# liuyuan-pal/Gen6D

Hardware: AMD Instinct MI355X
Metric: query images/sec (detect+select+3x refine), 64 ref views (higher is better)
Workload: dtype f32

## Files before the change

gen6d_amd/csrc/corr_fft.hip:

```cpp
#include "g6d_common.h"
#include "corr_fft_plan.h"

namespace {

constexpr int T = 32, HB = T / 2 + 1;
constexpr int CG = 32;
constexpr int RS = HB * 2 * CG;
constexpr int FWD_LDS = T * RS * 4;
constexpr int NT = 512;

struct CfftSeg { const float* in; float* out; int ld_in, ld_out; };
struct CfftParams {
  cfft::Plan plan;
  CfftSeg seg[cfft::MAX_SEG];
  int Cin;
  float* X;
  const float* Y;
};

__host__ __device__ constexpr double tw_c8(int k) {
  constexpr double c[9] = {1.0, 0.98078528040323043, 0.92387953251128674, 0.83146961230254524, 0.70710678118654752,
                           0.55557023301960218, 0.38268343236508977, 0.19509032201612825, 0.0};
  return c[k];
}
__host__ __device__ constexpr double tw_cos(int k) { return k <= 8 ? tw_c8(k) : -tw_c8(16 - k); }
__host__ __device__ constexpr double tw_sin(int k) { return k <= 8 ? tw_c8(8 - k) : tw_c8(k - 8); }
__host__ __device__ constexpr int br5(int k) { return ((k & 1) << 4) | ((k & 2) << 2) | (k & 4) | ((k & 8) >> 2) | ((k & 16) >> 4); }

__device__ __forceinline__ void fft32(float (&re)[T], float (&im)[T]) {
#pragma unroll
  for (int h = 16; h >= 1; h >>= 1) {
#pragma unroll
    for (int b = 0; b < T; b += 2 * h) {
#pragma unroll
      for (int j = 0; j < h; ++j) {
        const int k = j * (16 / h);
        const float c = (float)tw_cos(k), s = (float)tw_sin(k);
        const float ur = re[b + j], ui = im[b + j], vr = re[b + j + h], vi = im[b + j + h];
        re[b + j] = ur + vr; im[b + j] = ui + vi;
        const float dr = ur - vr, di = ui - vi;
        if (k == 0) { re[b + j + h] = dr; im[b + j + h] = di; }
        else if (k == 8) { re[b + j + h] = di; im[b + j + h] = -dr; }
        else { re[b + j + h] = dr * c + di * s; im[b + j + h] = di * c - dr * s; }
      }
    }
  }
}

__global__ __launch_bounds__(NT) void corrfft_fwd_kernel(const CfftParams p) {
  extern __shared__ __attribute__((aligned(16))) float L[];
  const int tid = threadIdx.x, c = tid & (CG - 1), g = tid >> 5;
  const int tile = blockIdx.x, c0 = blockIdx.y * CG;
  const cfft::Tile t = cfft::tile_of(p.plan, tile);
  const cfft::SegPlan& sp = p.plan.seg[t.seg];
  const CfftSeg& sg = p.seg[t.seg];
  const int H = sp.H, W = sp.W, wy = cfft::window_y(p.plan, t), wx = cfft::window_x(p.plan, t);
  float re[T], im[T];
  {
    const int ya = wy + 2 * g, yb = ya + 1;
    const bool oka = ya >= 0 && ya < H, okb = yb >= 0 && yb < H;
    const float* img = sg.in + (size_t)t.n * H * W * sg.ld_in + c0 + c;
#pragma unroll
    for (int x = 0; x < T; ++x) {
      const int xx = wx + x;
      const bool okx = xx >= 0 && xx < W;
      re[x] = oka && okx ? img[((size_t)ya * W + xx) * sg.ld_in] : 0.f;
      im[x] = okb && okx ? img[((size_t)yb * W + xx) * sg.ld_in] : 0.f;
    }
  }
  fft32(re, im);
  {
    float* ra = L + (2 * g) * RS + c;
    float* rb = ra + RS;
#pragma unroll
    for (int k = 0; k < HB; ++k) {
      const int a = br5(k), b = br5((T - k) & (T - 1));
      ra[k * 64] = 0.5f * (re[a] + re[b]); ra[k * 64 + 32] = 0.5f * (im[a] - im[b]);
      rb[k * 64] = 0.5f * (im[a] + im[b]); rb[k * 64 + 32] = 0.5f * (re[b] - re[a]);
    }
  }
  __syncthreads();
  if (g == 0) {
#pragma unroll
    for (int y = 0; y < T; ++y) { re[y] = L[y * RS + c]; im[y] = L[y * RS + 16 * 64 + c]; }
  } else {
#pragma unroll
    for (int y = 0; y < T; ++y) { re[y] = L[y * RS + g * 64 + c]; im[y] = L[y * RS + g * 64 + 32 + c]; }
  }
  fft32(re, im);
  if (g == 0) {
#pragma unroll
    for (int k = 0; k < T; ++k) {
      const int a = br5(k), b = br5((T - k) & (T - 1));
      L[k * RS + c] = 0.5f * (re[a] + re[b]); L[k * RS + 32 + c] = 0.5f * (im[a] - im[b]);
      L[k * RS + 16 * 64 + c] = 0.5f * (im[a] + im[b]); L[k * RS + 16 * 64 + 32 + c] = 0.5f * (re[b] - re[a]);
    }
  } else {
#pragma unroll
    for (int k = 0; k < T; ++k) { L[k * RS + g * 64 + c] = re[br5(k)]; L[k * RS + g * 64 + 32 + c] = im[br5(k)]; }
  }
  __syncthreads();
  const size_t tiles = (size_t)p.plan.tiles;
#pragma unroll 1
  for (int i = tid; i < T * HB * 16; i += NT) {
    const int q = i & 7, pl = (i >> 3) & 1, bin = i >> 4, ky = bin / HB, kx = bin - ky * HB;
    const f32x4 v = *reinterpret_cast<const f32x4*>(L + ky * RS + kx * 64 + pl * 32 + 4 * q);
    *reinterpret_cast<f32x4*>(p.X + (((size_t)bin * tiles + tile) * 2 + pl) * p.Cin + c0 + 4 * q) = v;
  }
}

constexpr int GEMM_NT = 128, GEMM_BM = 128;
struct CfftGemm { const float* X; const float* B; float* Y; int M, bins, K2, mblocks; };

__global__ __launch_bounds__(GEMM_NT) void corrfft_gemm_kernel(const CfftGemm p) {
  const int b = blockIdx.x, xcd = b & 7, s = b >> 3;
  const int bin = xcd + 8 * (s / p.mblocks), mb = s % p.mblocks;
  if (bin >= p.bins) return;
  const int lane = threadIdx.x & 63, wv = threadIdx.x >> 6, r = lane & 31, h = lane >> 5;
  const int m0 = mb * GEMM_BM + wv * 64;
  if (m0 >= p.M) return;
  const int K2 = p.K2;
  const float* A0 = p.X + ((size_t)bin * p.M + min(m0 + r, p.M - 1)) * K2 + 16 * h;
  const float* A1 = p.X + ((size_t)bin * p.M + min(m0 + 32 + r, p.M - 1)) * K2 + 16 * h;
  const float* Bp = p.B + ((size_t)bin * K2 + 16 * h) * 64 + r;
  f32x16 acc[2][2];
#pragma unroll
  for (int i = 0; i < 2; ++i)
#pragma unroll
    for (int n = 0; n < 2; ++n)
#pragma unroll
      for (int q = 0; q < 16; ++q) acc[i][n][q] = 0.f;
  f32x4 a0[2][4], a1[2][4];
  float b0[2][16], b1[2][16];
  auto load = [&](int k0, f32x4 (&x0)[4], f32x4 (&x1)[4], float (&y0)[16], float (&y1)[16]) {
#pragma unroll
    for (int j = 0; j < 4; ++j) {
      x0[j] = *reinterpret_cast<const f32x4*>(A0 + k0 + 4 * j);
      x1[j] = *reinterpret_cast<const f32x4*>(A1 + k0 + 4 * j);
    }
#pragma unroll
    for (int e = 0; e < 16; ++e) { y0[e] = Bp[(size_t)(k0 + e) * 64]; y1[e] = Bp[(size_t)(k0 + e) * 64 + 32]; }
  };
  auto mac = [&](const f32x4 (&x0)[4], const f32x4 (&x1)[4], const float (&y0)[16], const float (&y1)[16]) {
#pragma unroll
    for (int e = 0; e < 16; ++e) {
      const float u0 = x0[e >> 2][e & 3], u1 = x1[e >> 2][e & 3];
      acc[0][0] = __builtin_amdgcn_mfma_f32_32x32x2f32(u0, y0[e], acc[0][0], 0, 0, 0);
      acc[0][1] = __builtin_amdgcn_mfma_f32_32x32x2f32(u0, y1[e], acc[0][1], 0, 0, 0);
      acc[1][0] = __builtin_amdgcn_mfma_f32_32x32x2f32(u1, y0[e], acc[1][0], 0, 0, 0);
      acc[1][1] = __builtin_amdgcn_mfma_f32_32x32x2f32(u1, y1[e], acc[1][1], 0, 0, 0);
    }
  };
  load(0, a0[0], a1[0], b0[0], b1[0]);
#pragma unroll 1
  for (int k0 = 0; k0 < K2; k0 += 64) {
    load(k0 + 32, a0[1], a1[1], b0[1], b1[1]);
    mac(a0[0], a1[0], b0[0], b1[0]);
    if (k0 + 64 < K2) load(k0 + 64, a0[0], a1[0], b0[0], b1[0]);
    mac(a0[1], a1[1], b0[1], b1[1]);
  }
  float* Yb = p.Y + (size_t)bin * p.M * 64 + r;
#pragma unroll
  for (int i = 0; i < 2; ++i)
#pragma unroll
    for (int q = 0; q < 16; ++q) {
      const int row = m0 + 32 * i + (q & 3) + 8 * (q >> 2) + 4 * h;
      if (row < p.M) { Yb[(size_t)row * 64] = acc[i][0][q]; Yb[(size_t)row * 64 + 32] = acc[i][1][q]; }
    }
}

constexpr int INV_ROWS = 18;
constexpr int INV_LDS = INV_ROWS * RS * 4;

__global__ __launch_bounds__(NT) void corrfft_inv_kernel(const CfftParams p) {
  extern __shared__ __attribute__((aligned(16))) float L[];
  const int tid = threadIdx.x, r = tid & (CG - 1), g = tid >> 5;
  const int tile = blockIdx.x, V = p.plan.V;
  const cfft::Tile t = cfft::tile_of(p.plan, tile);
  const cfft::SegPlan& sp = p.plan.seg[t.seg];
  const CfftSeg& sg = p.seg[t.seg];
  const size_t bs = (size_t)p.plan.tiles * 64;
  const float* Y = p.Y + (size_t)tile * 64 + r;
  float re[T], im[T];
  if (g == 0) {
#pragma unroll
    for (int k = 0; k < T; ++k) {
      const float* y0 = Y + (size_t)(k * HB) * bs;
      const float* y16 = Y + (size_t)(k * HB + 16) * bs;
      re[k] = y0[0] - y16[32]; im[k] = y0[32] + y16[0];
    }
  } else {
#pragma unroll
    for (int k = 0; k < T; ++k) {
      const float* y = Y + (size_t)(k * HB + g) * bs;
      re[k] = y[0]; im[k] = y[32];
    }
  }
  fft32(im, re);
  if (g == 0) {
#pragma unroll
    for (int y = 0; y < INV_ROWS; ++y) {
      L[y * RS + r] = re[br5(y)]; L[y * RS + 32 + r] = 0.f;
      L[y * RS + 16 * 64 + r] = im[br5(y)]; L[y * RS + 16 * 64 + 32 + r] = 0.f;
    }
  } else {
#pragma unroll
    for (int y = 0; y < INV_ROWS; ++y) { L[y * RS + g * 64 + r] = re[br5(y)]; L[y * RS + g * 64 + 32 + r] = im[br5(y)]; }
  }
  __syncthreads();
  if (2 * g >= V) return;
  const float* ga = L + (2 * g) * RS + r;
  const float* gb = ga + RS;
#pragma unroll
  for (int k = 0; k < HB; ++k) {
    const float ar = ga[k * 64], ai = ga[k * 64 + 32], br = gb[k * 64], bi = gb[k * 64 + 32];
    re[k] = ar - bi; im[k] = ai + br;
    if (k > 0 && k < T / 2) { re[T - k] = ar + bi; im[T - k] = br - ai; }
  }
  fft32(im, re);
  const int H = sp.H, W = sp.W, ya = t.y0 + 2 * g;
  const float sc = 1.f / (T * T);
  float* o = sg.out + (size_t)t.n * H * W * sg.ld_out + r;
#pragma unroll
  for (int x = 0; x < INV_ROWS; ++x) {
    const int xx = t.x0 + x;
    if (x < V && xx < W) {
      if (ya < H) o[((size_t)ya * W + xx) * sg.ld_out] = re[br5(x)] * sc;
      if (ya + 1 < H) o[((size_t)(ya + 1) * W + xx) * sg.ld_out] = im[br5(x)] * sc;
    }
  }
}

int cfft_params(CfftParams& p, const char* what, const G6dCorrSeg* segs, int nseg, int C, int k, int Tw, bool fwd) {
  if (!segs || nseg < 1 || nseg > cfft::MAX_SEG) { g6d_set_error("corr_fft: 1..4 segments expected"); return G6D_EINVAL; }
  if (Tw != T || k != 15) { g6d_set_error("corr_fft: the kernels are built for T = 32, k = 15"); return G6D_EINVAL; }
  int N[cfft::MAX_SEG], H[cfft::MAX_SEG], W[cfft::MAX_SEG];
  for (int i = 0; i < nseg; ++i) { N[i] = segs[i].N; H[i] = segs[i].H; W[i] = segs[i].W; }
  if (!cfft::make_plan(p.plan, Tw, k, nseg, N, H, W) || p.plan.V > INV_ROWS || (p.plan.V & 1)) { g6d_set_error("corr_fft: bad map sizes"); return G6D_EINVAL; }
  for (int i = 0; i < nseg; ++i) {
    const G6dCorrSeg& s = segs[i];
    const bool ok = fwd ? (s.in && s.ld_in >= C && !(s.ld_in & 3) && g6d_aligned16(s.in)) : (s.out && s.ld_out >= C);
    if (!ok) { g6d_set_error(what); return G6D_EINVAL; }
    p.seg[i] = CfftSeg{s.in, s.out, s.ld_in, s.ld_out};
  }
  return G6D_OK;
}
}

extern "C" int g6d_corr_fft_plan(const G6dCorrSeg* segs, int nseg, int Cin, int Cout, int k, int Tw, int64_t* out) {
  if (!segs || !out || nseg < 1 || nseg > cfft::MAX_SEG || Cin < 1 || Cout < 1) { g6d_set_error("corr_fft_plan: bad arguments"); return G6D_EINVAL; }
  int N[cfft::MAX_SEG], H[cfft::MAX_SEG], W[cfft::MAX_SEG], one[cfft::MAX_SEG];
  for (int i = 0; i < nseg; ++i) { N[i] = segs[i].N; H[i] = segs[i].H; W[i] = segs[i].W; one[i] = 1; }
  cfft::Plan p, q;
  if (!cfft::make_plan(p, Tw, k, nseg, N, H, W) || !cfft::make_plan(q, Tw, k, nseg, one, H, W)) { g6d_set_error("corr_fft_plan: bad sizes"); return G6D_EINVAL; }
  out[0] = p.tiles; out[1] = p.bins; out[2] = p.V;
  out[3] = cfft::spectrum_bytes(Tw, p.tiles, Cin); out[4] = cfft::product_bytes(Tw, p.tiles, Cout); out[5] = cfft::filter_bytes(Tw, Cin, Cout);
  out[6] = q.tiles;
  out[7] = cfft::chunk_queries(Tw, q.tiles, Cin, 1 << 16);
  return G6D_OK;
}

extern "C" int g6d_corr_fft_fwd(const G6dCorrSeg* segs, int nseg, int Cin, int k, int Tw, float* X, g6d_stream_t stream) {
  CfftParams p = {};
  if (int rc = cfft_params(p, "corr_fft_fwd: bad segment (fp32 channels-last maps, 16-byte aligned, ld_in % 4 == 0)", segs, nseg, Cin, k, Tw, true)) return rc;
  if (!X || !g6d_aligned16(X) || Cin % CG) { g6d_set_error("corr_fft_fwd: Cin % 32 == 0 and an aligned spectrum expected"); return G6D_EINVAL; }
  if (cfft::spectrum_bytes(Tw, p.plan.tiles, Cin) >= (1ll << 31)) { g6d_set_error("corr_fft_fwd: spectrum beyond 2 GB, launch fewer queries"); return G6D_ENOSPC; }
  p.Cin = Cin; p.X = X;
  g6d_allow_lds(reinterpret_cast<const void*>(&corrfft_fwd_kernel), FWD_LDS);
  hipLaunchKernelGGL(corrfft_fwd_kernel, dim3(p.plan.tiles, Cin / CG), dim3(NT), FWD_LDS, static_cast<hipStream_t>(stream), p);
  return g6d_check_launch("corr_fft_fwd");
}

extern "C" int g6d_corr_fft_gemm(const float* X, const float* B, float* Y, int tiles, int Cin, int Cout, int Tw, g6d_stream_t stream) {
  if (!X || !B || !Y || tiles < 1 || Tw != T || Cout != 32 || Cin < 32 || Cin % 32 || !g6d_aligned16(X)) {
    g6d_set_error("corr_fft_gemm: T = 32, 32 references, Cin % 32 == 0 expected"); return G6D_EINVAL;
  }
  if (cfft::spectrum_bytes(Tw, tiles, Cin) >= (1ll << 31)) { g6d_set_error("corr_fft_gemm: spectrum beyond 2 GB"); return G6D_ENOSPC; }
  CfftGemm p = {X, B, Y, tiles, cfft::bins(Tw), 2 * Cin, (tiles + GEMM_BM - 1) / GEMM_BM};
  static_assert(cfft::bins(T) % 8 == 0, "blocks of a bin stay on one XCD");
  hipLaunchKernelGGL(corrfft_gemm_kernel, dim3(p.bins * p.mblocks), dim3(GEMM_NT), 0, static_cast<hipStream_t>(stream), p);
  return g6d_check_launch("corr_fft_gemm");
}

extern "C" int g6d_corr_fft_inv(const G6dCorrSeg* segs, int nseg, int Cout, int k, int Tw, const float* Y, g6d_stream_t stream) {
  CfftParams p = {};
  if (int rc = cfft_params(p, "corr_fft_inv: bad segment (ld_out >= 32)", segs, nseg, Cout, k, Tw, false)) return rc;
  if (!Y || Cout != CG) { g6d_set_error("corr_fft_inv: 32 references expected"); return G6D_EINVAL; }
  p.Y = Y;
  g6d_allow_lds(reinterpret_cast<const void*>(&corrfft_inv_kernel), INV_LDS);
  hipLaunchKernelGGL(corrfft_inv_kernel, dim3(p.plan.tiles), dim3(NT), INV_LDS, static_cast<hipStream_t>(stream), p);
  return g6d_check_launch("corr_fft_inv");
}
```

gen6d_amd/csrc/corr_fft_plan.h:

```cpp
#pragma once
#include <stdint.h>

#if defined(__HIPCC__) || defined(__CUDACC__)
#define CFFT_HD __host__ __device__ inline
#else
#define CFFT_HD inline
#endif

namespace cfft {

constexpr int MAX_SEG = 4;

CFFT_HD constexpr bool valid_tk(int T, int K) { return (T == 32 || T == 64) && K >= 1 && (K & 1) && K < T; }
CFFT_HD constexpr int valid_side(int T, int K) { return T - K + 1; }
CFFT_HD constexpr int bins(int T) { return T * (T / 2 + 1); }

struct SegPlan { int H, W, N, tiles_x, tiles_y, tpi, tile0; };
struct Plan {
  int T, K, V, bins, nseg, tiles;
  SegPlan seg[MAX_SEG];
};
struct Tile { int seg, n, y0, x0; };

CFFT_HD int ceil_div(int a, int b) { return (a + b - 1) / b; }

CFFT_HD bool make_plan(Plan& p, int T, int K, int nseg, const int* N, const int* H, const int* W) {
  if (!valid_tk(T, K) || nseg < 1 || nseg > MAX_SEG) return false;
  p.T = T; p.K = K; p.V = valid_side(T, K); p.bins = bins(T); p.nseg = nseg;
  int64_t tiles = 0;
  for (int i = 0; i < nseg; ++i) {
    if (N[i] < 1 || H[i] < 1 || W[i] < 1) return false;
    SegPlan& s = p.seg[i];
    s.H = H[i]; s.W = W[i]; s.N = N[i];
    s.tiles_x = ceil_div(W[i], p.V); s.tiles_y = ceil_div(H[i], p.V);
    s.tpi = s.tiles_x * s.tiles_y; s.tile0 = (int)tiles;
    tiles += (int64_t)s.tpi * N[i];
    if (tiles >= (1ll << 24)) return false;
  }
  p.tiles = (int)tiles;
  return true;
}

CFFT_HD Tile tile_of(const Plan& p, int t) {
  int si = 0;
  for (int i = 1; i < p.nseg; ++i) if (t >= p.seg[i].tile0) si = i;
  const SegPlan& s = p.seg[si];
  const int l = t - s.tile0, n = l / s.tpi, r = l - n * s.tpi, ty = r / s.tiles_x, tx = r - ty * s.tiles_x;
  return {si, n, ty * p.V, tx * p.V};
}
CFFT_HD int window_y(const Plan& p, const Tile& t) { return t.y0 - p.K / 2; }
CFFT_HD int window_x(const Plan& p, const Tile& t) { return t.x0 - p.K / 2; }

CFFT_HD int64_t spectrum_bytes(int T, int64_t tiles, int Cin) { return (int64_t)bins(T) * tiles * 2 * Cin * 4; }
CFFT_HD int64_t product_bytes(int T, int64_t tiles, int R) { return (int64_t)bins(T) * tiles * 2 * R * 4; }
CFFT_HD int64_t filter_bytes(int T, int Cin, int R) { return (int64_t)bins(T) * 2 * Cin * 2 * R * 4; }

CFFT_HD int chunk_queries(int T, int tiles_per_query, int Cin, int want) {
  int q = want;
  while (q > 0 && spectrum_bytes(T, (int64_t)q * tiles_per_query, Cin) >= (1ll << 31)) --q;
  return q;
}

}
```

gen6d_amd/ops.py:

```python
import ctypes as C
import math

import numpy as np
import torch

from . import lib as _lib

_WS = {}
WORKSPACE_BYTES = 96 << 20
MATH_MODE = 0
_MATH_NAMES = {"fp32": 0, "f32": 0, "bf16": 1, "fp16": 2, "f16": 2, 0: 0, 1: 1, 2: 2, None: 0}


class math_mode:

    def __init__(self, mode, inherit_if_none=False):
        self.mode = None if (mode is None and inherit_if_none) else _MATH_NAMES[mode]

    def __enter__(self):
        global MATH_MODE
        self.prev = MATH_MODE
        if self.mode is not None:
            MATH_MODE = self.mode
        return self
# ... 808 lines not shown
def l2norm_split16(x, mode, rng=None):
    _need_gpu(x)
    if x.dtype != torch.float32 or not x.is_contiguous() or x.dim() != 4:
        raise ValueError("l2norm_split16: a dense float32 [N,H,W,C] tap expected")
    N, H, W, Cc = x.shape
    out, ra = _pair_out("l2norm_split16", (N, H, W), Cc, mode, x.device, rng)
    _timed_hbm("l2norm_split16", 4.0 * x.numel() + 2.0 * out.numel(), lambda: _lib.check(_lib.load().g6d_l2norm_split16(
        _ptr(x), Cc, N * H * W, Cc, _ptr(out), int(mode), ra, _stream()), "g6d_l2norm_split16"))
    return _wrap(out, rng)


def vgg_conv1_pool_nhwc16(x, w_oihw, bias, out=None, norm=None, mode=None, rng=None):
    _need_gpu(x, w_oihw, bias)
    mode = MATH_MODE if mode is None else mode
    if mode not in _T16:
        raise RuntimeError("vgg_conv1_pool_nhwc16: mode 1 (bf16), 2 (fp16) or 3 (fp16 pairs)")
    N, Cin, H, W = x.shape
    Cout = w_oihw.shape[0]
    out, ra = _pair_out("vgg_conv1_pool_nhwc16", (N, H // 2, W // 2), Cout, mode, x.device, rng, out)
    mean = std = None
    if norm is not None:
        mean, std = (C.c_float * 3)(*norm[0]), (C.c_float * 3)(*norm[1])
    _lib.check(_lib.load().g6d_vgg_conv1_pool_nhwc16_ex(_ptr(x.contiguous()), N, H, W, _ptr(w_oihw.contiguous()), _ptr(bias), Cin, Cout,
                                                        mean, std, _ptr(out), int(mode), ra, _stream()),
               "g6d_vgg_conv1_pool_nhwc16")
    return _wrap(out, rng)


def conv16_direct_multi(xs, filt, bias, relu=True, full=None, pool=None, kd=1, stats=None, rows_per_group=0, out_full=None, rng=None):
    xs, table_in, slot_in = _pair_inputs(xs)
    if (table_in is not None or rng is not None) and filt.mode != 3:
        raise ValueError("conv16_direct_multi: ranges apply to pairs (mode 3) only")
    ra = _range_arg(table_in, slot_in, rng)
    _need_gpu(filt.data, *xs)
    mode = filt.mode
    t16 = _T16[mode]
    Cout, taps, Cin = filt.Cout, filt.taps, filt.Cin
    if taps != 9 * kd:
        raise ValueError("conv16_direct_multi: filters / kd mismatch")
    pair = mode == 3
    code = {None: 0, "t16": 3 if pair else 1, torch.float32: 2}
    if full not in code or pool not in code:
        raise ValueError('conv16_direct_multi: output types are None, torch.float32 or "t16"')
    segs = (_lib.G6dConv16Seg * len(xs))()
    fulls, pools, flops, sizes, nbytes = [], [], 0.0, [], 2.0 * filt.data.numel()
    nd = (4 if kd == 1 else 5) + (1 if pair else 0)
    for i, x in enumerate(xs):
        if x.dtype != t16 or not x.is_contiguous() or x.dim() != nd or x.shape[-1] != Cin or (pair and x.shape[-2] != 2):
            raise ValueError(f"conv16_direct_multi: input {i} must be a dense {t16} channels-last tensor with {Cin} channels{' in hi / lo planes' if pair else ''}")
        N, D, H, W = (x.shape[0], 1, x.shape[1], x.shape[2]) if kd == 1 else tuple(x.shape[:4])
        lead = (N, H, W) if kd == 1 else (N, D, H, W)

        def alloc(kind, lead_):
            if kind is None:
                return None
            if kind == "t16":
                return torch.empty(lead_ + ((2, Cout) if pair else (Cout,)), dtype=t16, device=x.device)
            return torch.empty(lead_ + (Cout,), dtype=torch.float32, device=x.device)
        q = alloc(pool, (N, H // 2, W // 2))
        ld_f = None
        if out_full is not None:
            f = out_full[i]
            want_t = torch.float32 if full is torch.float32 else t16
            nel = N * D * H * W * Cout * (2 if (pair and full == "t16") else 1)
            if full is None or f.dtype != want_t or f.numel() != nel or f.stride(-1) != 1:
                raise ValueError("conv16_direct_multi: out_full must hold the outputs' type and size")
            if not f.is_contiguous():
                ld_f = f.stride(-2)
                if full is not torch.float32 or f.shape[-1] != Cout or any(f.stride(d) != f.stride(d + 1) * f.shape[d + 1] for d in range(f.dim() - 2)):
                    raise ValueError("conv16_direct_multi: a strided out_full must be an fp32 channel slice of dense rows")
        else:
            f = alloc(full, lead)
        fulls.append(f); pools.append(q)
        ld = lambda t_: (2 * Cout if t_.dtype != torch.float32 and pair else Cout)
        segs[i] = _lib.G6dConv16Seg(in_=x.data_ptr(), out_full=f.data_ptr() if f is not None else None,
                                    out_pool=q.data_ptr() if q is not None else None, N=N, D=D, H=H, W=W, ld_in=(2 if pair else 1) * Cin,
                                    ld_full=(ld_f or ld(f)) if f is not None else 0, ld_pool=ld(q) if q is not None else 0)
        flops += 2.0 * N * D * H * W * Cout * taps * Cin
        nbytes += x.numel() * 2.0 + sum(t.numel() * t.element_size() for t in (f, q) if t is not None)
        sizes.append("x".join(str(v) for v in lead))
    _timed(PROFILE is not None,
           lambda: _lib.check(_lib.load().g6d_conv16_direct_multi_ex(
               segs, len(xs), Cin, _ptr(filt.data), int(filt.layout), float(filt.acc_scale), _ptr(bias), Cout, int(kd), int(bool(relu)), code[full],
               code[pool], int(mode), _ptr(stats), int(rows_per_group), ra, _stream()), "g6d_conv16_direct_multi"),
           lambda e0, e1: PROFILE.append((flops, e0, e1, f"{'conv16x3' if pair else 'conv16'} direct in={'+'.join(sizes)}x{Cin} out={Cout} k={'3x' if kd == 3 else ''}3x3"
                                          f"{' full' if full is not None else ''}{' pool' if pool is not None else ''}{' stats' if stats is not None else ''}", nbytes, flops)))
    if rng is not None:
        fulls = [_wrap(f, rng) if full == "t16" else f for f in fulls]
        pools = [_wrap(q, rng) if pool == "t16" else q for q in pools]
    return fulls, pools


def conv16_direct_plan(N, H, W, Cin, Cout, mode, stats_rows=0, full=torch.float32, D=None):
    pair = mode == 3
    code = {None: 0, "t16": 3 if pair else 1, torch.float32: 2}[full]
    any_ = 1 << 12
    ldf = 2 * Cout if code == 3 else Cout
    seg = (_lib.G6dConv16Seg * 1)(_lib.G6dConv16Seg(in_=any_, out_full=any_ if code else None, out_pool=None, N=N, D=D or 1, H=H, W=W,
                                                    ld_in=(2 if pair else 1) * Cin, ld_full=ldf if code else 0, ld_pool=0))
    rc = _lib.load().g6d_conv16_direct_plan(seg, 1, Cin, C.c_void_p(any_), 2 if D else 1, Cout, 3 if D else 1, code, 0, int(mode),
                                            C.c_void_p(any_ if stats_rows else 0), int(stats_rows))
    return rc if rc >= 0 else None


def corr16_pack(w_taps, mode):
    co, taps, ci = w_taps.shape
    if co != 32 or ci % 32:
        raise ValueError("corr16_pack: 32 references and Cin % 32 == 0 expected")
    acc_scale = 1.0
    if mode == 3:
        hi, lo, acc_scale = _split_hi_lo(w_taps)
        x = torch.stack([hi, lo], 0).reshape(2, 32, taps, ci // 16, 2, 8)
        x = x.permute(3, 2, 0, 4, 1, 5).contiguous()
    else:
        x = w_taps.to(_T16[mode]).reshape(32, taps, ci // 32, 2, 2, 8)
        x = x.permute(2, 1, 3, 4, 0, 5).contiguous()
    k = int(round(taps ** 0.5))
    f = Conv16Filters(x.reshape(-1), 1, mode, acc_scale, co, taps, ci)
    f.k = k
    return f


def corr16_multi(xs, filt, outs):
    xs, table_in, slot_in = _pair_inputs(xs)
    if table_in is not None and filt.mode != 3:
        raise ValueError("corr16_multi: PairMaps need pair filters (mode 3)")
    ra = _range_arg(table_in, slot_in, None)
    _need_gpu(filt.data, *xs, *outs)
    mode, Cin = filt.mode, filt.Cin
    pair = mode == 3
    segs = (_lib.G6dConv16Seg * len(xs))()
    flops, sizes, nbytes = 0.0, [], 2.0 * filt.data.numel()
    for i, (x, o) in enumerate(zip(xs, outs)):
        if x.dtype != _T16[mode] or not x.is_contiguous() or x.dim() != (5 if pair else 4) or x.shape[-1] != Cin or not o.is_contiguous() \
                or o.dtype != torch.float32 or o.shape[-1] != 32:
            raise ValueError("corr16_multi: dense 16-bit channels-last inputs and dense fp32 outputs with 32 channels expected")
        N, H, W = x.shape[0], x.shape[1], x.shape[2]
        if o.numel() != N * H * W * 32:
            raise ValueError("corr16_multi: output shape mismatch")
        segs[i] = _lib.G6dConv16Seg(in_=x.data_ptr(), out_full=o.data_ptr(), out_pool=None, N=N, D=1, H=H, W=W, ld_in=(2 if pair else 1) * Cin,
                                    ld_full=32, ld_pool=0)
        flops += 2.0 * N * H * W * 32 * filt.taps * Cin
        nbytes += x.numel() * 2.0 + o.numel() * 4.0
        sizes.append(f"{N}x{H}x{W}")
    _timed(PROFILE is not None,
           lambda: _lib.check(_lib.load().g6d_corr16_multi_ex(segs, len(xs), Cin, _ptr(filt.data), float(filt.acc_scale), 32, int(filt.k), int(mode), ra,
                                                             _stream()), "g6d_corr16_multi"),
           lambda e0, e1: PROFILE.append((flops, e0, e1, f"{'conv16x3' if pair else 'conv16'} corr in={'+'.join(sizes)}x{Cin} out=32 k={filt.k}x{filt.k}",
                                          nbytes, flops)))
    return outs


CORR_FFT_T = 32
CORR_FFT_CHUNK = 4


def _corr_fft_segs(xs, outs, Cin, what):
    n = len(xs if xs is not None else outs)
    if not 1 <= n <= 4:
        raise ValueError(f"{what}: 1..4 segments expected")
    segs = (_lib.G6dCorrSeg * n)()
    for i in range(n):
        x = xs[i] if xs is not None else None
        o = outs[i] if outs is not None else None
        for t, ch in ((x, Cin), (o, 32)):
            if t is not None and (t.dtype != torch.float32 or not t.is_contiguous() or t.dim() not in (4, 5) or t.shape[-1] != ch
                                  or (t.dim() == 5 and t.shape[1] != 1)):
                raise ValueError(f"{what}: dense fp32 channels-last maps [N,(1,)H,W,{ch}] expected")
        ref = x if x is not None else o
        N, H, W = ref.shape[0], ref.shape[-3], ref.shape[-2]
        if x is not None and o is not None and (o.shape[0], o.shape[-3], o.shape[-2]) != (N, H, W):
            raise ValueError(f"{what}: output shape mismatch")
        segs[i] = _lib.G6dCorrSeg(in_=x.data_ptr() if x is not None else None, out=o.data_ptr() if o is not None else None, H=H, W=W,
                                  ld_in=Cin, ld_out=32, N=N, reserved_=0)
    return segs


def corr_fft_plan(sizes, Cin, Cout=32, k=15, T=CORR_FFT_T):
    segs = (_lib.G6dCorrSeg * len(sizes))()
    for i, (N, H, W) in enumerate(sizes):
        segs[i] = _lib.G6dCorrSeg(in_=None, out=None, H=H, W=W, ld_in=Cin, ld_out=Cout, N=N, reserved_=0)
    out = (C.c_int64 * 8)()
    _lib.check(_lib.load().g6d_corr_fft_plan(segs, len(sizes), Cin, Cout, k, T, out), "g6d_corr_fft_plan")
    keys = ("tiles", "bins", "V", "spectrum_bytes", "product_bytes", "filter_bytes", "tiles_per_query", "max_queries")
    return dict(zip(keys, (int(v) for v in out)))


class CorrFftSpectra:

    def __init__(self, data, Cin, k, T):
        self.data, self.Cin, self.k, self.T = data, Cin, k, T


def corr_fft_spectra(w_taps, T=CORR_FFT_T):
    R, taps, Cin = w_taps.shape
    k = int(round(taps ** 0.5))
    if R != 32 or k * k != taps or k >= T:
        raise ValueError("corr_fft_spectra: [32, k*k, Cin] filters with k < T expected")
    w = w_taps.detach().to("cpu", torch.float64).reshape(R, k, k, Cin).permute(0, 3, 1, 2)
    Wf = torch.fft.rfft2(torch.nn.functional.pad(w, (0, T - k, 0, T - k)))
    Wr = Wf.real.permute(2, 3, 1, 0).reshape(-1, Cin, R)
    Wi = Wf.imag.permute(2, 3, 1, 0).reshape(-1, Cin, R)
    B = torch.cat([torch.cat([Wr, -Wi], 2), torch.cat([Wi, Wr], 2)], 1).to(torch.float32).contiguous()
    return CorrFftSpectra(B.to(w_taps.device), Cin, k, T)


def corr_fft_fwd(xs, X, k=15, T=CORR_FFT_T):
    Cin = xs[0].shape[-1]
    _need_gpu(X, *xs)
    segs = _corr_fft_segs(xs, None, Cin, "corr_fft_fwd")
    plan = corr_fft_plan([(s.N, s.H, s.W) for s in segs], Cin, 32, k, T)
    if X.dtype != torch.float32 or not X.is_contiguous() or X.numel() * 4 < plan["spectrum_bytes"]:
        raise ValueError("corr_fft_fwd: the spectrum buffer is smaller than [bins][tiles][2][Cin] fp32")
    _lib.check(_lib.load().g6d_corr_fft_fwd(segs, len(xs), Cin, k, T, _ptr(X), _stream()), "g6d_corr_fft_fwd")
    return X


def corr_fft_gemm(X, B, Y, tiles, Cin, T=CORR_FFT_T):
    _need_gpu(X, B, Y)
    bins = T * (T // 2 + 1)
    if X.numel() < bins * tiles * 2 * Cin or B.numel() != bins * 2 * Cin * 64 or Y.numel() < bins * tiles * 64 \
            or any(t.dtype != torch.float32 or not t.is_contiguous() for t in (X, B, Y)):
        raise ValueError("corr_fft_gemm: fp32 X [bins][tiles][2 Cin], B' [bins][2 Cin][64], Y [bins][tiles][64] expected")
    _lib.check(_lib.load().g6d_corr_fft_gemm(_ptr(X), _ptr(B), _ptr(Y), int(tiles), int(Cin), 32, T, _stream()), "g6d_corr_fft_gemm")
    return Y


def corr_fft_inv(Y, outs, k=15, T=CORR_FFT_T):
    _need_gpu(Y, *outs)
    segs = _corr_fft_segs(None, outs, 32, "corr_fft_inv")
    plan = corr_fft_plan([(s.N, s.H, s.W) for s in segs], 32, 32, k, T)
    if Y.dtype != torch.float32 or not Y.is_contiguous() or Y.numel() * 4 < plan["product_bytes"]:
        raise ValueError("corr_fft_inv: the product buffer is smaller than [bins][tiles][2][32] fp32")
    _lib.check(_lib.load().g6d_corr_fft_inv(segs, len(outs), 32, k, T, _ptr(Y), _stream()), "g6d_corr_fft_inv")
    return outs


def corr_fft_multi(xs, spectra, outs, chunk=None):
    Cin, k, T = spectra.Cin, spectra.k, spectra.T
    N = xs[0].shape[0]
    if any(x.shape[0] != N or x.shape[-1] != Cin for x in xs) or len(xs) != len(outs):
        raise ValueError("corr_fft_multi: every segment holds the same queries and Cin channels")
    _need_gpu(spectra.data, *xs, *outs)
    _corr_fft_segs(xs, outs, Cin, "corr_fft_multi")
    one = corr_fft_plan([(1, x.shape[-3], x.shape[-2]) for x in xs], Cin, 32, k, T)
    qc = min(N, one["max_queries"], int(chunk or CORR_FFT_CHUNK))
    if qc < 1:
        raise ValueError("corr_fft_multi: one query's spectrum passes 2^31 bytes")
    dev = xs[0].device
    tiles_max = one["tiles_per_query"] * qc
    bins = one["bins"]
    X = torch.empty(bins * tiles_max * 2 * Cin, dtype=torch.float32, device=dev)
    Y = torch.empty(bins * tiles_max * 64, dtype=torch.float32, device=dev)
    on = PROFILE is not None
    log2t = math.log2(T)
    for q0 in range(0, N, qc):
        q1 = min(N, q0 + qc)
        tiles = one["tiles_per_query"] * (q1 - q0)
        xc, oc = [x[q0:q1] for x in xs], [o[q0:q1] for o in outs]
        sizes = "+".join(f"{q1 - q0}x{x.shape[-3]}x{x.shape[-2]}" for x in xs)
        f_fft = 5.0 * T * log2t
        fl_fwd = tiles * Cin * (T / 2 + T / 2) * f_fft
        fl_gemm = 2.0 * bins * tiles * (2 * Cin) * 64
        fl_inv = tiles * 32 * (T / 2 + (T - k + 1) / 2) * f_fft
        act = sum(x.numel() for x in xc) * 4.0
        _timed(on, lambda: corr_fft_fwd(xc, X, k, T),
               lambda e0, e1: PROFILE.append((fl_fwd, e0, e1, f"corr_fft fwd in={sizes}x{Cin} T={T}", act + 4.0 * bins * tiles * 2 * Cin, fl_fwd)))
        _timed(on, lambda: corr_fft_gemm(X, spectra.data, Y, tiles, Cin, T),
               lambda e0, e1: PROFILE.append((fl_gemm, e0, e1, f"corr_fft gemm bins={bins} M={tiles} K={2 * Cin} N=64",
                                              4.0 * (bins * tiles * (2 * Cin + 64) + spectra.data.numel()), fl_gemm)))
        _timed(on, lambda: corr_fft_inv(Y, oc, k, T),
               lambda e0, e1: PROFILE.append((fl_inv, e0, e1, f"corr_fft inv out={sizes}x32 T={T}",
                                              4.0 * bins * tiles * 64 + sum(o.numel() for o in oc) * 4.0, fl_inv)))
    return outs


def l2norm_rows(x):
    _need_gpu(x)
    Cc = x.shape[-1]
    if x.dtype == torch.float32 and x.dim() == 2 and x.stride(1) == 1 and not x.is_contiguous():
        _lib.check(_lib.load().g6d_l2norm_rows(_ptr(x), x.shape[0], Cc, x.stride(0), _stream()), "g6d_l2norm_rows")
        return x
    if x.dtype != torch.float32 or not x.is_contiguous():
        raise ValueError("l2norm_rows: contiguous float32 expected")
    _lib.check(_lib.load().g6d_l2norm_rows(_ptr(x), x.numel() // Cc, Cc, Cc, _stream()), "g6d_l2norm_rows")
    return x


def nchw_to_nhwc(x, out, l2norm):
    _need_gpu(x, out)
    if not x.is_contiguous() or x.dtype != torch.float32:
        raise ValueError("nchw_to_nhwc: x must be contiguous float32 NCHW")
    N, Cc, H, W = x.shape
    _, _, Ho, Wo, Co, ld_out = _cl5(out, "nchw_to_nhwc.out")
    if (Ho, Wo, Co) != (H, W, Cc):
        raise ValueError("nchw_to_nhwc: shape mismatch")
    _lib.check(_lib.load().g6d_nchw_to_nhwc(_ptr(x), N, Cc, H, W, int(l2norm), _ptr(out), ld_out, _stream()), "g6d_nchw_to_nhwc")
    return out


def selector_ref_sums(refs):
    _need_gpu(refs)
    D, HW, Cc = refs.shape
    r1 = torch.empty((HW, Cc), dtype=torch.float64, device=refs.device)
    r2 = torch.empty_like(r1)
    _lib.check(_lib.load().g6d_selector_ref_sums(_ptr(refs.contiguous()), D, HW, Cc, _ptr(r1), _ptr(r2), _stream()),
               "g6d_selector_ref_sums")
# ... 592 lines not shown
```

Measured before the change: 391.4.

## Stage FFT-correlation GEMM operands through swizzled LDS with async buffer loads

The per-bin complex GEMM in the FFT correlation path now stages X and B' tiles into LDS with buffer_load-to-LDS in a multi-stage ring, rather than loading operands straight into registers from global memory. The A tile uses an XOR swizzle to avoid bank conflicts. Blocks are sized to 2 or 4 waves depending on M, with balanced rows per block and idle waves kept only for barrier participation. The query chunk size in Python also doubles. The aim is to hide global latency and coalesce B' loads, at the cost of LDS use, barriers and hand-written waitcnt logic.

```diff
diff --git a/gen6d_amd/csrc/corr_fft.hip b/gen6d_amd/csrc/corr_fft.hip
--- a/gen6d_amd/csrc/corr_fft.hip
+++ b/gen6d_amd/csrc/corr_fft.hip
@@ -109,20 +109,46 @@
   }
 }
 
-constexpr int GEMM_NT = 128, GEMM_BM = 128;
-struct CfftGemm { const float* X; const float* B; float* Y; int M, bins, K2, mblocks; };
-
-__global__ __launch_bounds__(GEMM_NT) void corrfft_gemm_kernel(const CfftGemm p) {
-  const int b = blockIdx.x, xcd = b & 7, s = b >> 3;
-  const int bin = xcd + 8 * (s / p.mblocks), mb = s % p.mblocks;
+struct CfftGemm { const float* X; const float* B; float* Y; int M, bins, K2, mblocks, rows; };
+typedef __attribute__((address_space(3))) void* cfft_lds_ptr;
+
+template <bool V> struct CfftBool { static constexpr bool value = V; };
+template <int N> __device__ __forceinline__ void cfft_wait_vm() { asm volatile("s_waitcnt vmcnt(%0)" ::"n"(N) : "memory"); }
+
+template <int WAVES, int STAGES>
+__global__ __launch_bounds__(WAVES * 64) void corrfft_gemm_kernel(const CfftGemm p) {
+  extern __shared__ __attribute__((aligned(16))) char gl[];
+  constexpr int ASTG = cfft::gemm_a_stage_bytes(WAVES), STG = cfft::gemm_stage_bytes(WAVES);
+  constexpr int PB = cfft::gemm_b_pieces_per_wave(WAVES);
+  constexpr int WIMG = cfft::GEMM_WAVE_ROWS * cfft::GEMM_ROW_BYTES;
+  static_assert(STAGES == cfft::gemm_stages(WAVES) && (STAGES == 2 || STAGES == 3), "the waits below are written for rings of two and three");
+  int bin, mb;
+  cfft::gemm_block_of(blockIdx.x, p.mblocks, bin, mb);
   if (bin >= p.bins) return;
-  const int lane = threadIdx.x & 63, wv = threadIdx.x >> 6, r = lane & 31, h = lane >> 5;
-  const int m0 = mb * GEMM_BM + wv * 64;
-  if (m0 >= p.M) return;
-  const int K2 = p.K2;
-  const float* A0 = p.X + ((size_t)bin * p.M + min(m0 + r, p.M - 1)) * K2 + 16 * h;
-  const float* A1 = p.X + ((size_t)bin * p.M + min(m0 + 32 + r, p.M - 1)) * K2 + 16 * h;
-  const float* Bp = p.B + ((size_t)bin * K2 + 16 * h) * 64 + r;
+  const int lane = threadIdx.x & 63, wv = __builtin_amdgcn_readfirstlane(threadIdx.x >> 6), r = lane & 31, h = lane >> 5;
+  const int m0 = cfft::gemm_wave_row0(mb, wv, p.rows), K2 = p.K2, nsteps = K2 / cfft::GEMM_KSTEP;
+  const bool active = !cfft::gemm_wave_idle(mb, wv, p.rows, p.M);
+  const auto rs_a = __builtin_amdgcn_make_buffer_rsrc(const_cast<float*>(p.X) + (size_t)bin * p.M * K2, 0, p.M * K2 * 4, 0x00020000);
+  const auto rs_b = __builtin_amdgcn_make_buffer_rsrc(const_cast<float*>(p.B) + (size_t)bin * K2 * cfft::GEMM_COLS, 0, K2 * cfft::GEMM_COLS * 4, 0x00020000);
+  unsigned aoff[cfft::GEMM_A_PIECES];
+#pragma unroll
+  for (int c = 0; c < cfft::GEMM_A_PIECES; ++c)
+    aoff[c] = (unsigned)min(m0 + cfft::gemm_a_src_row(c, lane), p.M - 1) * (unsigned)(K2 * 4) + 16u * cfft::gemm_a_src_seg(c, lane);
+  const unsigned boff = (unsigned)(wv * PB) * cfft::GEMM_PIECE + 16u * lane;
+
+  auto issue = [&](int t, int st, bool with_a) {
+    char* sa = gl + st * STG;
+    const unsigned ka = (unsigned)t * cfft::GEMM_ROW_BYTES, kb = (unsigned)t * cfft::GEMM_B_STAGE;
+    if (with_a)
+#pragma unroll
+      for (int c = 0; c < cfft::GEMM_A_PIECES; ++c)
+        __builtin_amdgcn_raw_ptr_buffer_load_lds(rs_a, (cfft_lds_ptr)(sa + wv * WIMG + c * cfft::GEMM_PIECE), 16, aoff[c] + ka, 0, 0, 0);
+#pragma unroll
+    for (int q = 0; q < PB; ++q)
+      __builtin_amdgcn_raw_ptr_buffer_load_lds(rs_b, (cfft_lds_ptr)(sa + ASTG + (wv * PB + q) * cfft::GEMM_PIECE), 16,
+                                               boff + q * cfft::GEMM_PIECE + kb, 0, 0, 0);
+  };
+
   f32x16 acc[2][2];
 #pragma unroll
   for (int i = 0; i < 2; ++i)
@@ -130,18 +156,23 @@
     for (int n = 0; n < 2; ++n)
 #pragma unroll
       for (int q = 0; q < 16; ++q) acc[i][n][q] = 0.f;
-  f32x4 a0[2][4], a1[2][4];
-  float b0[2][16], b1[2][16];
-  auto load = [&](int k0, f32x4 (&x0)[4], f32x4 (&x1)[4], float (&y0)[16], float (&y1)[16]) {
+  f32x4 x0[4], x1[4];
+  float y0[16], y1[16];
+  auto fetch = [&](int st) {
+    const char* sa = gl + st * STG + wv * WIMG;
+    const char* sb = gl + st * STG + ASTG + cfft::gemm_b_lds_offset(16 * h, r);
 #pragma unroll
     for (int j = 0; j < 4; ++j) {
-      x0[j] = *reinterpret_cast<const f32x4*>(A0 + k0 + 4 * j);
-      x1[j] = *reinterpret_cast<const f32x4*>(A1 + k0 + 4 * j);
-    }
-#pragma unroll
-    for (int e = 0; e < 16; ++e) { y0[e] = Bp[(size_t)(k0 + e) * 64]; y1[e] = Bp[(size_t)(k0 + e) * 64 + 32]; }
+      x0[j] = *reinterpret_cast<const f32x4*>(sa + cfft::gemm_a_lds_offset(r, 4 * h + j));
+      x1[j] = *reinterpret_cast<const f32x4*>(sa + cfft::gemm_a_lds_offset(32 + r, 4 * h + j));
+#pragma unroll
+      for (int e = 4 * j; e < 4 * j + 4; ++e) {
+        y0[e] = *reinterpret_cast<const float*>(sb + cfft::gemm_b_lds_offset(e, 0));
+        y1[e] = *reinterpret_cast<const float*>(sb + cfft::gemm_b_lds_offset(e, 32));
+      }
+    }
   };
-  auto mac = [&](const f32x4 (&x0)[4], const f32x4 (&x1)[4], const float (&y0)[16], const float (&y1)[16]) {
+  auto mac = [&]() {
 #pragma unroll
     for (int e = 0; e < 16; ++e) {
       const float u0 = x0[e >> 2][e & 3], u1 = x1[e >> 2][e & 3];
@@ -151,14 +182,28 @@
       acc[1][1] = __builtin_amdgcn_mfma_f32_32x32x2f32(u1, y1[e], acc[1][1], 0, 0, 0);
     }
   };
-  load(0, a0[0], a1[0], b0[0], b1[0]);
+
+#pragma unroll
+  for (int t = 0; t < STAGES - 1; ++t) issue(t, t, active);
+  auto run = [&](auto act) {
+    constexpr int LOADS = cfft::gemm_loads_per_stage(WAVES, !decltype(act)::value);
+    int st = 0;
 #pragma unroll 1
-  for (int k0 = 0; k0 < K2; k0 += 64) {
-    load(k0 + 32, a0[1], a1[1], b0[1], b1[1]);
-    mac(a0[0], a1[0], b0[0], b1[0]);
-    if (k0 + 64 < K2) load(k0 + 64, a0[0], a1[0], b0[0], b1[0]);
-    mac(a0[1], a1[1], b0[1], b1[1]);
-  }
+    for (int t = 0; t < nsteps; ++t) {
+      if (cfft::gemm_ahead(STAGES, t, nsteps) == 1) cfft_wait_vm<LOADS>(); else cfft_wait_vm<0>();
+      asm volatile("s_waitcnt lgkmcnt(0)" ::: "memory");
+      __builtin_amdgcn_s_barrier();
+      __builtin_amdgcn_sched_barrier(0);
+      if (decltype(act)::value) { fetch(st); __builtin_amdgcn_sched_barrier(0); }
+      const int sn = st == 0 ? STAGES - 1 : st - 1;
+      if (t + STAGES - 1 < nsteps) issue(t + STAGES - 1, sn, decltype(act)::value);
+      __builtin_amdgcn_sched_barrier(0);
+      if (decltype(act)::value) mac();
+      st = st + 1 == STAGES ? 0 : st + 1;
+    }
+  };
+  if (!active) { run(CfftBool<false>{}); return; }
+  run(CfftBool<true>{});
   float* Yb = p.Y + (size_t)bin * p.M * 64 + r;
 #pragma unroll
   for (int i = 0; i < 2; ++i)
@@ -167,6 +212,13 @@
       const int row = m0 + 32 * i + (q & 3) + 8 * (q >> 2) + 4 * h;
       if (row < p.M) { Yb[(size_t)row * 64] = acc[i][0][q]; Yb[(size_t)row * 64 + 32] = acc[i][1][q]; }
     }
+}
+
+template <int WAVES>
+void cfft_gemm_launch(const CfftGemm& p, hipStream_t stream) {
+  constexpr int STAGES = cfft::gemm_stages(WAVES), LDS = cfft::gemm_lds_bytes(WAVES);
+  g6d_allow_lds(reinterpret_cast<const void*>(&corrfft_gemm_kernel<WAVES, STAGES>), LDS);
+  hipLaunchKernelGGL((corrfft_gemm_kernel<WAVES, STAGES>), dim3(p.bins * p.mblocks), dim3(WAVES * 64), LDS, stream, p);
 }
 
 constexpr int INV_ROWS = 18;
@@ -276,9 +328,11 @@
     g6d_set_error("corr_fft_gemm: T = 32, 32 references, Cin % 32 == 0 expected"); return G6D_EINVAL;
   }
   if (cfft::spectrum_bytes(Tw, tiles, Cin) >= (1ll << 31)) { g6d_set_error("corr_fft_gemm: spectrum beyond 2 GB"); return G6D_ENOSPC; }
-  CfftGemm p = {X, B, Y, tiles, cfft::bins(Tw), 2 * Cin, (tiles + GEMM_BM - 1) / GEMM_BM};
+  if (!g6d_aligned16(B)) { g6d_set_error("corr_fft_gemm: the filter spectrum is staged in 16-byte pieces, a 16-byte aligned B' expected"); return G6D_EINVAL; }
+  const CfftGemm p = {X, B, Y, tiles, cfft::bins(Tw), 2 * Cin, cfft::gemm_mblocks(tiles), cfft::gemm_rows_per_block(tiles)};
   static_assert(cfft::bins(T) % 8 == 0, "blocks of a bin stay on one XCD");
-  hipLaunchKernelGGL(corrfft_gemm_kernel, dim3(p.bins * p.mblocks), dim3(GEMM_NT), 0, static_cast<hipStream_t>(stream), p);
+  if (cfft::gemm_waves(tiles) == 2) cfft_gemm_launch<2>(p, static_cast<hipStream_t>(stream));
+  else cfft_gemm_launch<4>(p, static_cast<hipStream_t>(stream));
   return g6d_check_launch("corr_fft_gemm");
 }
 
diff --git a/gen6d_amd/csrc/corr_fft_plan.h b/gen6d_amd/csrc/corr_fft_plan.h
--- a/gen6d_amd/csrc/corr_fft_plan.h
+++ b/gen6d_amd/csrc/corr_fft_plan.h
@@ -61,4 +61,53 @@
   return q;
 }
 
+constexpr int GEMM_KSTEP = 32;
+constexpr int GEMM_WAVE_ROWS = 64;
+constexpr int GEMM_COLS = 64;
+constexpr int GEMM_PIECE = 1024;
+constexpr int GEMM_ROW_BYTES = GEMM_KSTEP * 4;
+constexpr int GEMM_SLOTS = GEMM_ROW_BYTES / 16;
+constexpr int GEMM_A_PIECES = GEMM_WAVE_ROWS * GEMM_ROW_BYTES / GEMM_PIECE;
+constexpr int GEMM_B_STAGE = GEMM_KSTEP * GEMM_COLS * 4;
+constexpr int GEMM_B_PIECES = GEMM_B_STAGE / GEMM_PIECE;
+constexpr int GEMM_SMALL_M = 128;
+constexpr int LDS_LIMIT = 160 * 1024;
+
+CFFT_HD constexpr int gemm_waves(int M) { return M <= GEMM_SMALL_M ? 2 : 4; }
+CFFT_HD constexpr int gemm_stages(int waves) { return waves == 2 ? 2 : 2; }
+CFFT_HD constexpr int gemm_block_rows(int waves) { return waves * GEMM_WAVE_ROWS; }
+CFFT_HD constexpr int gemm_a_stage_bytes(int waves) { return gemm_block_rows(waves) * GEMM_ROW_BYTES; }
+CFFT_HD constexpr int gemm_stage_bytes(int waves) { return gemm_a_stage_bytes(waves) + GEMM_B_STAGE; }
+CFFT_HD constexpr int gemm_lds_bytes(int waves) { return gemm_stages(waves) * gemm_stage_bytes(waves); }
+CFFT_HD constexpr int gemm_b_pieces_per_wave(int waves) { return GEMM_B_PIECES / waves; }
+CFFT_HD constexpr int gemm_loads_per_stage(int waves, bool idle = false) { return (idle ? 0 : GEMM_A_PIECES) + gemm_b_pieces_per_wave(waves); }
+CFFT_HD constexpr int gemm_mblocks(int M) { return (M + gemm_block_rows(gemm_waves(M)) - 1) / gemm_block_rows(gemm_waves(M)); }
+CFFT_HD constexpr int gemm_rows_per_block(int M) { return GEMM_WAVE_ROWS * ((M + gemm_mblocks(M) * GEMM_WAVE_ROWS - 1) / (gemm_mblocks(M) * GEMM_WAVE_ROWS)); }
+CFFT_HD constexpr int gemm_steps(int Cin) { return 2 * Cin / GEMM_KSTEP; }
+CFFT_HD constexpr int gemm_stage_of(int stages, int t) { return t % stages; }
+CFFT_HD constexpr int gemm_ahead(int stages, int t, int nsteps) { return nsteps - 1 - t < stages - 2 ? nsteps - 1 - t : stages - 2; }
+
+static_assert(GEMM_A_PIECES == 8 && GEMM_B_PIECES == 8 && GEMM_SLOTS == 8, "a piece is 8 rows x 8 slots");
+static_assert(GEMM_B_PIECES % 2 == 0 && GEMM_B_PIECES % 4 == 0, "B' pieces split evenly over the waves");
+static_assert(gemm_a_stage_bytes(2) + GEMM_B_STAGE == gemm_stage_bytes(2) && gemm_stage_bytes(4) == 4 * 8192 + 8192, "stage = X image + B' slab");
+static_assert(gemm_lds_bytes(2) * 3 <= LDS_LIMIT && gemm_lds_bytes(4) * 2 <= LDS_LIMIT, "three small or two large blocks fit the CU's LDS");
+static_assert(gemm_loads_per_stage(2) * (gemm_stages(2) - 1) < 64 && gemm_loads_per_stage(4) * (gemm_stages(4) - 1) < 64, "vmcnt has six bits");
+static_assert(gemm_block_rows(gemm_waves(GEMM_SMALL_M)) >= GEMM_SMALL_M, "a small bin is one block");
+static_assert(gemm_rows_per_block(292) == 192 && gemm_rows_per_block(584) == 256 && gemm_rows_per_block(73) == 128 && gemm_rows_per_block(257) == 192, "whole waves");
+
+CFFT_HD void gemm_block_of(int b, int mblocks, int& bin, int& mb) {
+  const int xcd = b & 7, s = b >> 3;
+  bin = xcd + 8 * (s / mblocks); mb = s % mblocks;
 }
+CFFT_HD constexpr int gemm_wave_row0(int mb, int wave, int rows_per_block) { return mb * rows_per_block + wave * GEMM_WAVE_ROWS; }
+CFFT_HD constexpr bool gemm_wave_idle(int mb, int wave, int rows_per_block, int M) {
+  return wave * GEMM_WAVE_ROWS >= rows_per_block || gemm_wave_row0(mb, wave, rows_per_block) >= M;
+}
+
+CFFT_HD constexpr int gemm_a_swz(int row) { return (row >> 1) & (GEMM_SLOTS - 1); }
+CFFT_HD constexpr int gemm_a_src_row(int piece, int lane) { return piece * 8 + (lane >> 3); }
+CFFT_HD constexpr int gemm_a_src_seg(int piece, int lane) { return (lane & 7) ^ gemm_a_swz(gemm_a_src_row(piece, lane)); }
+CFFT_HD constexpr int gemm_a_lds_offset(int row, int seg) { return row * GEMM_ROW_BYTES + ((seg ^ gemm_a_swz(row)) << 4); }
+CFFT_HD constexpr int gemm_b_lds_offset(int k, int col) { return (k * GEMM_COLS + col) * 4; }
+
+}
diff --git a/gen6d_amd/ops.py b/gen6d_amd/ops.py
--- a/gen6d_amd/ops.py
+++ b/gen6d_amd/ops.py
@@ -984,7 +984,7 @@
 
 
 CORR_FFT_T = 32
-CORR_FFT_CHUNK = 4
+CORR_FFT_CHUNK = 8
 
 
 def _corr_fft_segs(xs, outs, Cin, what):
```

After: 397.2 (median of 6 runs). 1.5% higher.
